# refresh-bio/KMC

Measured on NVIDIA H100. Metric: stage-2 k-mers/s (k=31), higher is better.
Workload: dtype u64

## Files before the change

kmc_b200/csrc/expand.cuh:

```cuda
#pragma once
#include "common.cuh"

#ifndef KMCB200_EXPAND_UNROLL
#define KMCB200_EXPAND_UNROLL 8
#endif

namespace kmcb {

constexpr int kExpandUnroll = KMCB200_EXPAND_UNROLL;

#ifndef KMCB200_EXPAND_IPT
#define KMCB200_EXPAND_IPT 8
#endif
template <int WORDS> struct ExpandCfg { static constexpr int kTile = WORDS == 1 ? 4096 : 2048, kThreads = WORDS == 1 ? 4096 / KMCB200_EXPAND_IPT : 256; };
constexpr int kExpandMinTile = 2048;

struct ExpandArgs {
	const uint8_t* bin;
	uint64_t size;
	const uint64_t* pack_start;
	uint32_t n_packs;
	uint32_t k;
	uint32_t min_rec_bytes;
	uint32_t tile;
	uint32_t both_strands;
	uint64_t n_rec;
	uint32_t* sk_off;
	uint32_t* sk_kpre;
	uint32_t* tile_first;
	uint32_t* pack_nsk;
	uint32_t* pack_nk;
	uint64_t* pack_kbase;
	uint32_t* pack_tbase;
	uint32_t* tile_pack;
	uint4* tile_desc;
	uint64_t tile_pack_cap;
	uint32_t* status;
	uint32_t* flags;
	void* recs;
	uint16_t* cells1;
	uint64_t* item_lo1;
	uint16_t* item_cnt1;
	uint32_t top_shift;
	uint32_t mode;
	uint32_t fshift, fprefix, fmask;
	uint64_t* hist12;
	unsigned long long* out_counter;
	const uint16_t* blk_of_prefix;
	const uint64_t* region_start;
	uint32_t n_blocks;
};
enum : uint32_t { kExpandAll = 0, kExpandCount12 = 1, kExpandFilter = 2, kExpandScatter = 3 };
constexpr uint32_t kExpandMaxBlocks = 512;
constexpr uint64_t kExpandUnknownRecs = ~0ull;

enum : uint32_t { kErrPackWalk = 1, kErrRecCount = 2 };
constexpr uint32_t kExpandAbortFlag = 2;

__device__ __forceinline__ uint64_t tile_first_base(uint64_t pack_start, uint32_t p, uint32_t tile) { return pack_start * 4 / tile + p; }

constexpr int kWalkSegBytes = 256;
constexpr int kWalkSegs = 256;
constexpr int kWalkChunk = kWalkSegBytes * kWalkSegs;
#ifndef KMCB200_WALK_SPEC
#define KMCB200_WALK_SPEC 1024
#endif
constexpr int kWalkSpec = KMCB200_WALK_SPEC;

__global__ void __launch_bounds__(kWalkSegs, 3) walk_packs_parallel_kernel(const ExpandArgs a, uint32_t* pack_done)
{
	extern __shared__ __align__(16) uint8_t wsm[];
	__shared__ uint32_t s_entry[kWalkSegs], s_exit[kWalkSegs], s_w[16];
	__shared__ uint32_t s_bad;
	const uint32_t p = blockIdx.x, tid = threadIdx.x, lane = tid & 31, warp = tid >> 5;
	const uint64_t pstart = a.pack_start[p];
	const uint32_t len = (uint32_t)min(a.pack_start[p + 1] - pstart, (uint64_t)kWalkChunk + 1);
	if (len > (uint32_t)kWalkChunk || len == 0) { if (tid == 0) pack_done[p] = len == 0 ? 1u : 0u; if (len == 0 && tid == 0) { a.pack_nsk[p] = 0; a.pack_nk[p] = 0; } return; }
	{
		const uintptr_t g0 = reinterpret_cast<uintptr_t>(a.bin + pstart);
		const uintptr_t g0a = g0 & ~(uintptr_t)15;
		const uint32_t shift = (uint32_t)(g0 - g0a);
		const uint32_t nvec = (len + shift + 15) >> 4;
		for (uint32_t v0 = tid; v0 < nvec; v0 += 8 * kWalkSegs) {
			uint4 r[8];
#pragma unroll
// ... 329 lines not shown
}

template <int WORDS>
__device__ __forceinline__ uint32_t rec_top_digit(const Rec<WORDS>& r, uint32_t shift)
{
	const uint32_t wi = shift >> 6, off = shift & 63u;
	uint64_t lo = r.w[0], hi = 0;
#pragma unroll
	for (int i = 1; i < WORDS; ++i) {
		if (wi == (uint32_t)i) lo = r.w[i];
		if (wi + 1 == (uint32_t)i) hi = r.w[i];
	}
	uint64_t v = lo >> off;
	if (WORDS > 1 && off) v |= hi << (64u - off);
	return (uint32_t)v & 0xFFu;
}

template <int WORDS>
__device__ __forceinline__ uint32_t msd_free_bits(const Rec<WORDS>& r, uint32_t shift, uint32_t mask)
{
	if (WORDS == 1) return (uint32_t)(r.w[0] >> shift) & mask;
	const uint32_t wi = shift >> 6, off = shift & 63u;
	uint64_t lo = r.w[0], hi = 0;
#pragma unroll
	for (int i = 1; i < WORDS; ++i) {
		if (wi == (uint32_t)i) lo = r.w[i];
		if (wi + 1 == (uint32_t)i) hi = r.w[i];
	}
	uint64_t v = lo >> off;
	if (off) v |= hi << (64u - off);
	return (uint32_t)v & mask;
}

template <int WORDS, uint32_t MODE = kExpandAll>
__global__ void __launch_bounds__(ExpandCfg<WORDS>::kThreads, WORDS <= 2 ? 2048 / ExpandCfg<WORDS>::kThreads : 6) expand_kernel(const ExpandArgs a)
{
	constexpr int kExpandTile = ExpandCfg<WORDS>::kTile, kExpandThreads = ExpandCfg<WORDS>::kThreads;
	constexpr int IPT = kExpandTile / kExpandThreads;
	constexpr int MAXSK = 1024, STAGE = 12288;
	constexpr int HW = kExpandTile / 32;
	__shared__ uint32_t hbits[HW];
	__shared__ uint32_t hpre[HW];
	__shared__ uint32_t s_bit[MAXSK];
	__shared__ __align__(16) uint8_t s_bytes[STAGE + 32];
	__shared__ uint32_t s_jmax;
	__shared__ unsigned long long s_fbase;
	__shared__ uint32_t warp_max[kExpandThreads / 32];
	__shared__ uint32_t htop[256];
	static_assert(HW <= 128 && HW % 32 == 0, "the head bitmap is scanned by one warp, HW / 32 words per lane");
	const uint32_t tid = threadIdx.x, lane = tid & 31, warp = tid >> 5;
	const uint32_t le_mask = 0xffffffffu >> (31u - lane);
	static_assert(kExpandThreads % 32 == 0, "output slot i * threads + tid belongs to lane tid % 32");
	if (tid < 256) htop[tid] = 0;
	const uint32_t total_tiles = a.status[1];
	Rec<WORDS>* __restrict__ out = reinterpret_cast<Rec<WORDS>*>(a.recs);

	for (uint32_t g = blockIdx.x; g < total_tiles; g += gridDim.x) {
		const uint4 da = __ldg(a.tile_desc + 2 * (size_t)g), db = __ldg(a.tile_desc + 2 * (size_t)g + 1);
		if (g + gridDim.x < total_tiles) asm volatile("prefetch.global.L2 [%0];" ::"l"(a.tile_desc + 2 * (size_t)(g + gridDim.x)));
		const uint64_t slot0 = da.x;
		const uint32_t nsk = da.y;
		const uint32_t j_lo = da.z;
		const uint32_t off_lo = da.w;
		const uint32_t tile_start = db.x & ~(uint32_t)(kExpandTile - 1);
		const uint32_t cnt = (db.x & (uint32_t)(kExpandTile - 1)) + 1u;
		const uint32_t* __restrict__ kpre = a.sk_kpre + slot0;
		const uint32_t* __restrict__ off = a.sk_off + slot0;
		const uintptr_t g0a = reinterpret_cast<uintptr_t>(a.bin + off_lo) & ~(uintptr_t)15;
		const uint32_t base_off = (uint32_t)(reinterpret_cast<uintptr_t>(a.bin + off_lo) - g0a);

		__syncthreads();
		if (tid < (uint32_t)HW) hbits[tid] = 0;
		if (tid == 0) s_jmax = j_lo;
		__syncthreads();
		{
			uint32_t jm = j_lo;
			for (uint32_t j = j_lo + tid; j < nsk; j += kExpandThreads) {
				const uint32_t kp = kpre[j];
				if (j > j_lo && kp >= tile_start + cnt) break;
				const uint32_t rel = j - j_lo;
				if (rel < (uint32_t)MAXSK) s_bit[rel] = 8u * (base_off + (off[j] - off_lo) + 1u) + 2u * tile_start - 2u * kp;
				if (j > j_lo) atomicOr(&hbits[(kp - tile_start) >> 5], 1u << ((kp - tile_start) & 31u));
				jm = j;
			}
			if (jm > j_lo) atomicMax(&s_jmax, jm);
		}
		__syncthreads();
		const uint32_t j_hi = s_jmax;
		const uint64_t b_hi = j_hi + 1 < nsk ? (uint64_t)off[j_hi + 1] : (uint64_t)db.y;
		const uint64_t span = reinterpret_cast<uintptr_t>(a.bin + b_hi) - g0a;
		const bool staged = (j_hi - j_lo) < (uint32_t)MAXSK && span + 16 <= (uint64_t)STAGE;
		if (staged)
			for (uint32_t v = tid; v * 16 < span + 8; v += kExpandThreads) {
				uint4 x = __ldg(reinterpret_cast<const uint4*>(g0a) + v);
				x.x = __byte_perm(x.x, 0, 0x0123); x.y = __byte_perm(x.y, 0, 0x0123); x.z = __byte_perm(x.z, 0, 0x0123); x.w = __byte_perm(x.w, 0, 0x0123);
				reinterpret_cast<uint4*>(s_bytes)[v] = x;
			}
		if (warp == 0) {
			constexpr int WPL = HW / 32;
			uint32_t c[WPL], tot = 0;
#pragma unroll
			for (int i = 0; i < WPL; ++i) { c[i] = __popc(hbits[lane * WPL + i]); tot += c[i]; }
			uint32_t inc = tot;
#pragma unroll
			for (int o = 1; o < 32; o <<= 1) {
				const uint32_t x = __shfl_up_sync(0xffffffffu, inc, o);
				if (lane >= (uint32_t)o) inc += x;
			}
			uint32_t ex = inc - tot;
#pragma unroll
			for (int i = 0; i < WPL; ++i) { hpre[lane * WPL + i] = ex; ex += c[i]; }
		}
		__syncthreads();

		const uint64_t obase = ((uint64_t)db.w << 32) | db.z;
		auto kmer_of = [&](uint32_t slot) -> Rec<WORDS> {
			const uint32_t rel = hpre[slot >> 5] + __popc(hbits[slot >> 5] & le_mask);
			if (staged) return extract_kmer_be32<WORDS>(reinterpret_cast<const uint32_t*>(s_bytes), s_bit[rel] + 2u * slot, a.k, a.both_strands != 0);
			const uint32_t j = j_lo + rel;
			const uint32_t s = tile_start + slot - kpre[j];
			return extract_kmer<WORDS>(a.bin + off[j] + 1, s, a.k, a.both_strands != 0,
				[](uintptr_t wa) { return __ldg(reinterpret_cast<const unsigned long long*>(wa)); });
		};
		if constexpr (MODE == kExpandAll) {
#pragma unroll kExpandUnroll
			for (int i = 0; i < IPT; ++i) {
				const uint32_t slot = i * kExpandThreads + tid;
				if (slot < cnt) {
					const Rec<WORDS> r = kmer_of(slot);
					out[obase + slot] = r;
					atomicAdd(&htop[rec_top_digit<WORDS>(r, a.top_shift)], 1u);
				}
			}
			__syncthreads();
			if (tid < 256) {
				a.cells1[(uint64_t)tid * total_tiles + g] = (uint16_t)htop[tid];
				htop[tid] = 0;
			}
			if (tid == 0) { a.item_lo1[g] = obase; a.item_cnt1[g] = (uint16_t)cnt; }
		} else if constexpr (MODE == kExpandCount12) {
			for (int i = 0; i < IPT; ++i) {
				const uint32_t slot = i * kExpandThreads + tid;
				if (slot < cnt) {
					const Rec<WORDS> r = kmer_of(slot);
					atomicAdd(reinterpret_cast<unsigned long long*>(a.hist12) + msd_free_bits<WORDS>(r, a.fshift, 0xFFFu), 1ull);
				}
			}
		} else if constexpr (MODE == kExpandScatter) {
			__shared__ uint32_t s_bcnt[kExpandMaxBlocks];
			__shared__ unsigned long long s_bbase[kExpandMaxBlocks];
			for (uint32_t b = tid; b < a.n_blocks; b += kExpandThreads) s_bcnt[b] = 0;
			__syncthreads();
			uint16_t blk[IPT], rnk[IPT];
#pragma unroll
			for (int i = 0; i < IPT; ++i) {
				const uint32_t slot = i * kExpandThreads + tid;
				if (slot < cnt) {
					const Rec<WORDS> r = kmer_of(slot);
					blk[i] = a.blk_of_prefix[msd_free_bits<WORDS>(r, a.fshift, 0xFFFu)];
					if (blk[i] != 0xFFFFu) rnk[i] = (uint16_t)atomicAdd(&s_bcnt[blk[i]], 1u);
				}
			}
			__syncthreads();
			for (uint32_t b = tid; b < a.n_blocks; b += kExpandThreads) {
				const uint32_t c = s_bcnt[b];
				if (c) s_bbase[b] = a.region_start[b] + atomicAdd(a.out_counter + b, (unsigned long long)c);
			}
			__syncthreads();
#pragma unroll
			for (int i = 0; i < IPT; ++i) {
				const uint32_t slot = i * kExpandThreads + tid;
				if (slot < cnt && blk[i] != 0xFFFFu) out[s_bbase[blk[i]] + rnk[i]] = kmer_of(slot);
// ... 25 lines not shown
```

kmc_b200/csrc/kmc_b200.cu:

```cuda
#include "../../include/kmc_b200.h"
#include "common.cuh"
#include "expand.cuh"
#include "expand_fused.cuh"
#include "radix_sort.cuh"
#include "count.cuh"
#include "msd_sort.cuh"
#include "leaf_warp.cuh"
#include "leaf_hash.cuh"
#include "leaf_hash_cta.cuh"
#include "leaf_hash_wide.cuh"
#include "split.cuh"
#include "fastx.cuh"
#include "small_k.cuh"

#include <cmath>
#include <cstddef>
#include <cstdarg>
#include <cstdio>
#include <cstdlib>
#include <cstring>
#include <string>
#include <vector>
#include <algorithm>
#include <list>
#include <thread>

using namespace kmcb;

namespace {

constexpr int kMaxPasses = 4 * 8;
constexpr int kHistRows = kMaxPasses + 1;
constexpr int kCounterSlots = kMaxPasses + 8;
constexpr uint32_t kEpochLimit = (1u << 22) - 2;
constexpr int kStageRing = 4;
constexpr size_t kMaxLeaves = 256 * 1024;
constexpr uint32_t kHeavyListCap = 2048;

thread_local std::string g_create_error;

enum { kHistNone = 0, kHistTiles = 1, kHistAligned = 2 };

struct ZeroBlock {
	uint64_t hist[kHistRows][256];
	uint32_t counters[kCounterSlots];
	uint32_t status[2];
	uint32_t msd_flags[4];
	uint32_t msd_n_items[2];
	uint32_t msd_counters[4];
	uint32_t pack_ticket[4];
	uint32_t heavy_count[2];
	uint32_t heavy_list[kHeavyListCap];
	uint32_t leaf_group_sum[kMaxLeaves / 1024];
};

static_assert(sizeof(ZeroBlock) % 4 == 0, "zeroed word by word");

struct Slot {
	cudaStream_t stream = nullptr;
	uint8_t* recs_a = nullptr; size_t recs_a_cap = 0;
	uint8_t* recs_b = nullptr; size_t recs_b_cap = 0;
	uint8_t* recs_x = nullptr; size_t recs_x_cap = 0;
	uint8_t* d_bin = nullptr; size_t bin_cap = 0;
	uint64_t* d_pack_start = nullptr; size_t packs_cap = 0;
	uint64_t* h_pack_start[kStageRing] = {}; cudaEvent_t ev_pack[kStageRing] = {}; int ring = 0;
	uint32_t* pack_nsk = nullptr; uint32_t* pack_nk = nullptr; uint32_t* pack_tbase = nullptr; uint64_t* pack_kbase = nullptr;
	uint32_t* pack_done = nullptr;
	uint32_t* sk_off = nullptr; size_t sk_off_cap = 0;
	uint32_t* sk_kpre = nullptr; size_t sk_kpre_cap = 0;
	uint32_t* tile_first = nullptr; size_t tile_first_cap = 0;
	uint32_t* tile_pack = nullptr; size_t tile_pack_cap = 0;
	uint4* tile_desc = nullptr; size_t tile_desc_cap = 0;
	ZeroBlock* zero = nullptr;
	uint64_t* desc = nullptr; size_t desc_cap = 0;
	uint64_t* msd_seg1 = nullptr;
	uint64_t* msd_start2 = nullptr;
	uint64_t* msd_start3 = nullptr;
	uint32_t* msd_item_base1 = nullptr;
	uint32_t* msd_item_base2 = nullptr;
	uint32_t* msd_item_seg2 = nullptr; size_t msd_item_seg2_cap = 0;
	uint64_t* msd_item_lo1 = nullptr; size_t msd_item_lo1_cap = 0;
	uint16_t* msd_item_cnt1 = nullptr; size_t msd_item_cnt1_cap = 0;
	uint16_t* msd_cells = nullptr; size_t msd_cells_cap = 0;
	uint32_t* msd_cell_scan = nullptr; size_t msd_cell_scan_cap = 0;
	uint32_t* msd_block_sums = nullptr; size_t msd_block_sums_cap = 0;
	uint8_t* leaf_tmp = nullptr; size_t leaf_tmp_cap = 0;
	uint32_t* leaf_emit = nullptr; uint64_t* leaf_off = nullptr;
	const char* pass_names[kMaxPasses + 8] = {};
	uint32_t last_n_packs = 1;
	uint64_t* cdesc = nullptr; size_t cdesc_cap = 0;
	uint64_t* pdesc = nullptr; size_t pdesc_cap = 0;
	int hist_mode = 0;
	uint8_t* d_out = nullptr; size_t out_cap = 0;
	uint64_t* d_lut = nullptr;
	uint64_t* d_result = nullptr; uint64_t* h_result = nullptr; uint64_t* h_result_dev = nullptr;
	cudaEvent_t ev_begin = nullptr, ev_expand = nullptr, ev_sort = nullptr, ev_count = nullptr, ev_result = nullptr;
	cudaEvent_t ev_h2d = nullptr, ev_done = nullptr, ev_walk = nullptr;
	cudaEvent_t ev_pass[kMaxPasses + 8] = {};
	int n_passes_run = 0;
	bool ran_expand = false, ran_sort = false, ran_count = false;
	uint64_t* d_hist12 = nullptr; unsigned long long* d_out_counter = nullptr; size_t out_counter_cap = 0;
	uint16_t* d_blk_of_prefix = nullptr; uint64_t* d_region_start = nullptr; size_t region_cap = 0; bool last_scatter = false;
	uint64_t* tot_lut = nullptr; uint64_t* tot_res = nullptr; uint32_t last_blocks = 0;
	bool scan_lut = false; uint64_t scan_base = 0;
	uint8_t* d_extras = nullptr; size_t extras_cap = 0; uint64_t* d_pack_rec = nullptr; size_t pack_rec_cap = 0;
	uint64_t* h_pack_rec = nullptr; size_t h_pack_rec_cap = 0; bool have_extras = false;
	bool sync_done = false; uint64_t sync_out_bytes = 0; uint64_t sync_stats[4] = {};
	bool busy = false;
	uint8_t* host_out = nullptr; uint64_t host_out_cap = 0; uint64_t* host_lut = nullptr; uint64_t pending_n_rec = 0;
};

}

struct kmcb200_ctx {
	kmcb200_params prm{};
	int words = 1;
	uint32_t key_bytes = 0, suffix_bytes = 0, counter_bytes = 0;
	uint64_t lut_entries = 0;
	int sm_count = 0;
	int occ_radix = 1, occ_expand = 1, occ_msd_part = 1, occ_msd_part_wide = 1, occ_msd_local = 1;
	uint32_t force_b2 = 0;
	bool use_msd = true;
	bool use_fused = false;
	bool scatter_blocks = true;
	uint64_t key_block_records = 1ull << 28;
	bool overlap_walk = true;
	bool use_leaf = true;
	int occ_leaf = 1;
	int occ_leaf_hash = 1;
	bool leaf_hash_wide = true;
	bool leaf_hash = true;
	int leaf_cta = 2;
	int leaf_cta_warps = 4, leaf_cta_slot_bits = 12;
	int occ_leaf_cta = 1;
	uint32_t leaf_max_b2 = 8;
	uint32_t leaf_target = 1024;
	uint32_t leaf_fill_pct = 62;
	uint32_t leaf_ratio0_q8 = 90;
	uint64_t max_block_records = 1ull << 28;
	uint64_t max_chunk_bytes = 1ull << 30;
	uint32_t leaf_round_pct = 100;
	int leaf_slot_bits = 10;
	uint32_t epoch = 1;
	uint64_t launches = 0;
	cudaStream_t compute = nullptr;
	std::vector<Slot> slots;
	std::string err;
};

namespace {

int fail(kmcb200_ctx* c, int code, const char* fmt, ...)
{
// ... 53 lines not shown
	size_t n = std::max<size_t>(need_elems + need_elems / 8, 1024);
	if (p) CU(cudaFree(p));
	p = nullptr; cap = 0;
	CU(cudaMalloc(reinterpret_cast<void**>(&p), n * sizeof(T) + 256));
	if (zero) { CU(cudaMemset(p, 0, n * sizeof(T) + 256)); CU(cudaDeviceSynchronize()); }
	cap = n;
	return 0;
}

int next_epoch(kmcb200_ctx* ctx, uint32_t* out, uint32_t count = 1)
{
	if (ctx->epoch + count >= kEpochLimit) {
		CU(cudaDeviceSynchronize());
		for (auto& s : ctx->slots) {
			if (s.desc) CU(cudaMemset(s.desc, 0, s.desc_cap * sizeof(uint64_t)));
			if (s.cdesc) CU(cudaMemset(s.cdesc, 0, s.cdesc_cap * sizeof(uint64_t)));
			if (s.pdesc) CU(cudaMemset(s.pdesc, 0, s.pdesc_cap * sizeof(uint64_t)));
		}
		CU(cudaDeviceSynchronize());
		ctx->epoch = 1;
	}
	*out = ctx->epoch;
	ctx->epoch += count;
	return 0;
}

template <int WORDS>
int setup_kernels(kmcb200_ctx* ctx)
{
	CU(cudaFuncSetAttribute(radix_pass_kernel<WORDS>, cudaFuncAttributeMaxDynamicSharedMemorySize, SortSmem<WORDS>::kBytes));
	CU(cudaFuncSetAttribute(lsd_sort_kernel<WORDS>, cudaFuncAttributeMaxDynamicSharedMemorySize, SortSmem<WORDS>::kBytes));
	CU(cudaOccupancyMaxActiveBlocksPerMultiprocessor(&ctx->occ_radix, lsd_sort_kernel<WORDS>, SortCfg<WORDS>::kThreads, SortSmem<WORDS>::kBytes));
	CU(cudaOccupancyMaxActiveBlocksPerMultiprocessor(&ctx->occ_expand, expand_kernel<WORDS>, ExpandCfg<WORDS>::kThreads, 0));
	CU(cudaFuncSetAttribute(expand_fused_kernel<WORDS>, cudaFuncAttributeMaxDynamicSharedMemorySize, FxSmem<WORDS>::kBytes));
	const size_t cs = count_smem_bytes<WORDS>(ctx->suffix_bytes + ctx->counter_bytes);
	CU(cudaFuncSetAttribute(count_emit_kernel<WORDS>, cudaFuncAttributeMaxDynamicSharedMemorySize, (int)cs));
	CU(cudaFuncSetAttribute(msd_partition_kernel<WORDS>, cudaFuncAttributeMaxDynamicSharedMemorySize, MsdSmem<WORDS>::kBytes));
	CU(cudaOccupancyMaxActiveBlocksPerMultiprocessor(&ctx->occ_msd_part, msd_partition_kernel<WORDS>, MsdCfg<WORDS>::kThreads + 32, MsdSmem<WORDS>::kBytes));
	CU(cudaFuncSetAttribute(msd_partition_kernel<WORDS, 1024>, cudaFuncAttributeMaxDynamicSharedMemorySize, MsdSmem<WORDS, 1024>::kBytes));
	CU(cudaOccupancyMaxActiveBlocksPerMultiprocessor(&ctx->occ_msd_part_wide, msd_partition_kernel<WORDS, 1024>, MsdCfg<WORDS>::kThreads + 32, MsdSmem<WORDS, 1024>::kBytes));
	if (ctx->occ_msd_part_wide < 1) ctx->occ_msd_part_wide = 1;
	const int local_smem = msd_local_cap<WORDS>() * 8 * WORDS + (MsdLocalCfg<WORDS>::kThreads / 32) * 1024;
	CU(cudaFuncSetAttribute(msd_local_sort_kernel<WORDS>, cudaFuncAttributeMaxDynamicSharedMemorySize, local_smem));
	CU(cudaOccupancyMaxActiveBlocksPerMultiprocessor(&ctx->occ_msd_local, msd_local_sort_kernel<WORDS>, MsdLocalCfg<WORDS>::kThreads, local_smem));
	if (ctx->occ_radix < 1) ctx->occ_radix = 1;
	if (ctx->occ_expand < 1) ctx->occ_expand = 1;
	if (ctx->occ_msd_part < 1) ctx->occ_msd_part = 1;
	if (ctx->occ_msd_local < 1) ctx->occ_msd_local = 1;
	return 0;
}

template <int WORDS>
int launch_expand(kmcb200_ctx* ctx, const ExpandArgs& a, cudaStream_t st)
{
	const uint64_t n_bound = a.n_rec == kExpandUnknownRecs ? a.size * 4 : a.n_rec;
	const uint32_t max_tiles = (uint32_t)(n_bound / ExpandCfg<WORDS>::kTile) + a.n_packs + 1;
	const uint32_t grid = std::min<uint32_t>(max_tiles, (uint32_t)(ctx->sm_count * ctx->occ_expand));
	switch (a.mode) {
	case kExpandAll: expand_kernel<WORDS, kExpandAll><<<grid, ExpandCfg<WORDS>::kThreads, 0, st>>>(a); break;
	case kExpandCount12: expand_kernel<WORDS, kExpandCount12><<<grid, ExpandCfg<WORDS>::kThreads, 0, st>>>(a); break;
	case kExpandScatter: expand_kernel<WORDS, kExpandScatter><<<grid, ExpandCfg<WORDS>::kThreads, 0, st>>>(a); break;
	default: expand_kernel<WORDS, kExpandFilter><<<grid, ExpandCfg<WORDS>::kThreads, 0, st>>>(a); break;
	}
	ctx->launches++;
	CU(cudaGetLastError());
	return 0;
}

__global__ void msd_setup_kernel(uint64_t* seg1, uint32_t* item_base1, uint32_t* n_items1, uint64_t n, uint32_t tile)
{
	seg1[0] = 0; seg1[1] = n;
	const uint32_t nt = (uint32_t)((n + tile - 1) / tile);
	item_base1[0] = 0; item_base1[1] = nt;
	*n_items1 = nt;
}

template <int WORDS>
uint32_t choose_b2(const kmcb200_ctx* ctx, uint64_t n, bool counted_leaves)
{
	auto bits_for = [&](uint64_t target) { uint32_t lg = 0; while ((1ull << lg) < (n + target - 1) / target) ++lg; return lg > 8 ? lg - 8 : 0u; };
	uint32_t b2;
	if (counted_leaves) {
		b2 = std::min(bits_for(1024), 10u);
		if (WORDS == 1 && b2 > 8 && !ctx->leaf_hash) b2 = std::max(8u, std::min(bits_for(2048), 10u));
		if (WORDS == 1 && b2 > 8 && ctx->leaf_hash) b2 = std::max(8u, std::min(bits_for(ctx->leaf_target), ctx->leaf_max_b2));
		if (ctx->force_b2) b2 = ctx->force_b2;
	} else
		b2 = std::min(bits_for(std::max<uint64_t>(msd_local_cap<WORDS>() / 5, 64)), 8u);
	return b2;
}
template <int WORDS> uint32_t choose_nd2(const kmcb200_ctx* ctx, uint64_t n, bool counted_leaves) { return 1u << choose_b2<WORDS>(ctx, n, counted_leaves); }

// ... 21 lines not shown
	cell_reduce_kernel<<<nb, 256, 0, st>>>(s.msd_cells, n_items, nd, s.msd_block_sums, flags);
	cell_scan_sums_kernel<<<1, 1024, 0, st>>>(s.msd_block_sums, n_items, nd, flags);
	cell_scan_kernel<<<nb, 256, 0, st>>>(s.msd_cells, n_items, nd, s.msd_block_sums, s.msd_cell_scan, flags);
	ctx->launches += 3;
	CU(cudaGetLastError());
	return 0;
}

template <int WORDS>
int launch_lsd_sort(kmcb200_ctx* ctx, Slot& s, void* in, void* out, uint64_t n, uint32_t key_bytes, const uint32_t* run_flag, uint32_t run_need,
	uint64_t* reset_lut, uint64_t* reset_result, cudaStream_t st)
{
	constexpr int TILE = SortSmem<WORDS>::kTile;
	LsdSortArgs a{};
	a.a = in; a.b = out; a.n = n; a.n_tiles = (uint32_t)((n + TILE - 1) / TILE); a.key_bytes = key_bytes;
	a.hist = &s.zero->hist[0][0]; a.desc = s.desc; a.tile_counters = s.zero->counters;
	if (int rc = next_epoch(ctx, &a.epoch0, key_bytes)) return rc;
	a.run_flag = run_flag; a.run_need = run_need;
	a.reset_lut = reset_lut; a.reset_lut_entries = ctx->lut_entries; a.reset_result = reset_result;
	const uint32_t grid = std::max(1u, std::min<uint32_t>(a.n_tiles, (uint32_t)(ctx->sm_count * ctx->occ_radix)));
	void* params[] = {&a};
	CU(cudaLaunchCooperativeKernel(reinterpret_cast<const void*>(lsd_sort_kernel<WORDS>), dim3(grid), dim3(SortCfg<WORDS>::kThreads), params, SortSmem<WORDS>::kBytes, st));
	ctx->launches++;
	return 0;
}

struct LeafPlan {
	bool active = false;
	const void* recs = nullptr;
	const uint64_t* start = nullptr;
	uint32_t n_leaves = 0, low_bits = 0;
};

template <int WORDS>
int launch_sort(kmcb200_ctx* ctx, Slot& s, void* a, void* b, uint64_t n, uint32_t key_bytes, uint32_t key_bits, int hist_mode, uint32_t n_packs, cudaStream_t st, bool* result_in_b, LeafPlan* plan = nullptr)
{
	constexpr int TILE = SortSmem<WORDS>::kTile;
	constexpr int MTILE = msd_tile<WORDS>();
	const uint64_t n_tiles64 = (n + TILE - 1) / TILE;
	if (n_tiles64 > 0x7fffffffull || n >= (1ull << 32)) return fail(ctx, KMCB200_ERR_INVALID, "bin too large: %llu records", (unsigned long long)n);
	const uint32_t n_tiles = (uint32_t)n_tiles64;
	const bool msd = ctx->use_msd && key_bits >= 24 && n >= (1u << 16);
	const uint32_t top_shift = key_bits - 8;
	if (int rc = ensure(ctx, s.desc, s.desc_cap, (size_t)n_tiles * 256, true)) return rc;
	if (msd) if (int rc = ensure_msd<WORDS>(ctx, s, n, n_packs, choose_nd2<WORDS>(ctx, n, plan != nullptr))) return rc;

	const bool hist_ready = hist_mode == kHistTiles;
	if (hist_mode == kHistNone) if (int rc = zero_async(ctx, s.zero, sizeof(ZeroBlock), st)) return rc;
	int iv = 0;
	CU(cudaEventRecord(s.ev_pass[0], st));
	void* lsd_in = a; void* lsd_out = b;
	const uint32_t* lsd_flag = nullptr;
	if (msd) {
		const uint32_t b2 = choose_b2<WORDS>(ctx, n, plan != nullptr);
		const uint32_t nd2 = 1u << b2;
		const uint32_t cap = plan ? (WORDS == 1 ? kLwMaxHeavyLeaf : kLwMaxLeaf) : (uint32_t)msd_local_cap<WORDS>();
		const bool final_in_b = (key_bytes % 2) == 0;
		void* fin = final_in_b ? b : a;
		uint32_t* flags = s.zero->msd_flags;
		const uint32_t* never = &flags[1];
		const size_t max_items1 = hist_ready ? msd_max_items1(n, n_packs) : (size_t)(n / MTILE) + 2;
		const size_t max_items2 = (size_t)(n / MTILE) + 260;
		const uint32_t pgrid1 = (uint32_t)std::min<size_t>(max_items1, (size_t)ctx->sm_count * ctx->occ_msd_part);
		const uint32_t pgrid2 = (uint32_t)std::min<size_t>(max_items2, (size_t)ctx->sm_count * (nd2 > 256 ? ctx->occ_msd_part_wide : ctx->occ_msd_part));
		const int local_smem = msd_local_cap<WORDS>() * 8 * WORDS + (MsdLocalCfg<WORDS>::kThreads / 32) * 1024;

		MsdItems items1{};
		if (hist_ready) {
			items1.item_lo = s.msd_item_lo1; items1.item_cnt = s.msd_item_cnt1; items1.n_items = &s.zero->status[1];
		} else if (hist_mode == kHistAligned) {
			items1.seg_start = s.msd_seg1; items1.item_base = s.msd_item_base1; items1.item_seg = s.msd_item_seg2; items1.n_items = s.msd_item_base1 + 1;
		} else {
			msd_setup_kernel<<<1, 1, 0, st>>>(s.msd_seg1, s.msd_item_base1, &s.zero->msd_n_items[0], n, MTILE);
			items1.seg_start = s.msd_seg1; items1.item_base = s.msd_item_base1; items1.item_seg = s.msd_item_seg2 ;
			items1.n_items = &s.zero->msd_n_items[0];
			if (int rc = zero_async(ctx, s.msd_item_seg2, max_items1 * sizeof(uint32_t), st)) return rc;
			MsdCountArgs c1{a, items1, top_shift, 256, s.msd_cells, never};
			msd_count_kernel<WORDS><<<(uint32_t)std::min<size_t>(max_items1, (size_t)ctx->sm_count * 4), 512, 0, st>>>(c1);
			ctx->launches += 2;
		}
		if (int rc = launch_cell_scan(ctx, s, items1.n_items, 256, max_items1, never, st)) return rc;
		s.pass_names[iv] = "msd_scan_L1"; CU(cudaEventRecord(s.ev_pass[++iv], st));
		MsdBoundsArgs b1{};
		b1.cell_scan = s.msd_cell_scan; b1.items = items1; b1.S = 1; b1.nd = 256; b1.n = n; b1.start = s.msd_start2;
		b1.cap = b2 == 0 ? cap : 0; b1.flags = flags;
		b1.tile = b2 > 0 ? MTILE : 0; b1.item_base = s.msd_item_base2; b1.item_seg = s.msd_item_seg2; b1.n_items = &s.zero->msd_n_items[1];
		MsdPartArgs p1{};
		p1.in = a; p1.out = b; p1.items = items1; p1.cell_scan = s.msd_cell_scan; p1.shift = top_shift; p1.nd = 256;
		p1.flags = never;
		msd_partition_kernel<WORDS><<<pgrid1, MsdCfg<WORDS>::kThreads + 32, MsdSmem<WORDS>::kBytes, st>>>(p1);
		s.pass_names[iv] = "msd_partition_L1"; CU(cudaEventRecord(s.ev_pass[++iv], st));
		msd_bounds_kernel<<<1, 1024, 0, st>>>(b1);
		ctx->launches += 2;
		if (b2 > 0) {
			MsdItems items2{};
			items2.seg_start = s.msd_start2; items2.item_base = s.msd_item_base2; items2.item_seg = s.msd_item_seg2; items2.n_items = &s.zero->msd_n_items[1];
			MsdCountArgs c2{b, items2, top_shift - b2, nd2, s.msd_cells, flags};
			if (nd2 > 512) msd_count_kernel<WORDS, 1024><<<(uint32_t)std::min<size_t>(max_items2, (size_t)ctx->sm_count * 4), 512, 0, st>>>(c2);
			else if (nd2 > 256) msd_count_kernel<WORDS, 512><<<(uint32_t)std::min<size_t>(max_items2, (size_t)ctx->sm_count * 4), 512, 0, st>>>(c2);
			else msd_count_kernel<WORDS><<<(uint32_t)std::min<size_t>(max_items2, (size_t)ctx->sm_count * 4), 512, 0, st>>>(c2);
			ctx->launches++;
			if (int rc = launch_cell_scan(ctx, s, items2.n_items, nd2, max_items2, flags, st)) return rc;
			MsdBoundsArgs bb{};
			bb.cell_scan = s.msd_cell_scan; bb.items = items2; bb.S = 256; bb.nd = nd2; bb.n = n; bb.start = s.msd_start3; bb.cap = cap; bb.flags = flags; bb.tile = 0;
			msd_bounds_flat_kernel<<<(256 * nd2 + 256) / 256 + 1, 256, 0, st>>>(bb);
			ctx->launches++;
			s.pass_names[iv] = "msd_count_L2"; CU(cudaEventRecord(s.ev_pass[++iv], st));
			MsdPartArgs p2{};
			p2.in = b; p2.out = a; p2.items = items2; p2.cell_scan = s.msd_cell_scan; p2.shift = top_shift - b2; p2.nd = nd2;
			p2.flags = flags;
			if (nd2 > 256) msd_partition_kernel<WORDS, 1024><<<pgrid2, MsdCfg<WORDS>::kThreads + 32, MsdSmem<WORDS, 1024>::kBytes, st>>>(p2);
			else msd_partition_kernel<WORDS><<<pgrid2, MsdCfg<WORDS>::kThreads + 32, MsdSmem<WORDS>::kBytes, st>>>(p2);
			ctx->launches++;
			s.pass_names[iv] = "msd_partition_L2"; CU(cudaEventRecord(s.ev_pass[++iv], st));
		}
		if (plan) {
			plan->active = true;
			plan->recs = b2 > 0 ? a : b; plan->start = b2 > 0 ? s.msd_start3 : s.msd_start2; plan->n_leaves = 256 * nd2; plan->low_bits = top_shift - b2;
		} else {
			MsdLocalArgs lo{};
			lo.in = b2 > 0 ? a : b; lo.out = fin; lo.start = b2 > 0 ? s.msd_start3 : s.msd_start2; lo.n_buckets = 256 * nd2;
			lo.low_bits = top_shift - b2; lo.bucket_counter = &s.zero->msd_counters[2]; lo.flags = flags;
			const uint32_t lgrid = (uint32_t)std::min<size_t>(lo.n_buckets, (size_t)ctx->sm_count * ctx->occ_msd_local);
			msd_local_sort_kernel<WORDS><<<lgrid, MsdLocalCfg<WORDS>::kThreads, local_smem, st>>>(lo);
			ctx->launches++;
			s.pass_names[iv] = "msd_local_sort"; CU(cudaEventRecord(s.ev_pass[++iv], st));
// ... 115 lines not shown
	if (fused) {
		st = st_expand;
		const uint32_t nd2 = DISPATCH_WORDS(ctx, choose_nd2, ctx, n_rec, ctx->use_leaf);
		if (int rc = DISPATCH_WORDS(ctx, ensure_msd, ctx, s, n_rec, np, nd2)) return rc;
		if (int rc = ensure(ctx, s.pdesc, s.pdesc_cap, (size_t)np + 1, true)) return rc;
		const uint32_t mtile = ctx->words == 1 ? (uint32_t)msd_tile<1>() : (uint32_t)msd_tile<2>();
		static_assert(msd_tile<2>() == msd_tile<3>() && msd_tile<2>() == msd_tile<4>(), "one tile size for all wide records");
		const uint32_t n_tiles = (uint32_t)((n_rec + mtile - 1) / mtile);
		uint32_t tile_shift = 0;
		while ((1u << tile_shift) < mtile) ++tile_shift;
		InitExtra x;
		x.cells = reinterpret_cast<uint32_t*>(s.msd_cells); x.cell_words = ((size_t)256 * n_tiles + 1) / 2;
		x.item_seg = s.msd_item_seg2; x.item_seg_words = (size_t)n_tiles + 2;
		x.seg1 = s.msd_seg1; x.item_base1 = s.msd_item_base1; x.n = n_rec; x.n_tiles = n_tiles;
		bin_init_kernel<<<296, 256, 0, st>>>(reinterpret_cast<uint32_t*>(s.zero), (uint32_t)(sizeof(ZeroBlock) / 4), reinterpret_cast<uint32_t*>(zero_lut),
			(size_t)ctx->lut_entries * 2, reinterpret_cast<uint32_t*>(zero_result), x);
		FusedArgs f{};
		f.bin = d_bin; f.size = size; f.pack_start = s.d_pack_start; f.n_packs = np; f.k = k; f.both_strands = ctx->prm.both_strands; f.n_rec = n_rec;
		f.recs = d_recs; f.cells1 = reinterpret_cast<uint32_t*>(s.msd_cells); f.n_tiles = n_tiles; f.tile_shift = tile_shift;
		f.top_shift = std::max(2u * k, 8u) - 8u;
		f.desc = s.pdesc; f.ticket = &s.zero->pack_ticket[0]; f.status = s.zero->status; f.flags = s.zero->msd_flags;
		if (int rc = next_epoch(ctx, &f.epoch)) return rc;
		switch (ctx->words) {
		case 1: expand_fused_kernel<1><<<np, kFxThreads, FxSmem<1>::kBytes, st>>>(f); break;
		case 2: expand_fused_kernel<2><<<np, kFxThreads, FxSmem<2>::kBytes, st>>>(f); break;
		case 3: expand_fused_kernel<3><<<np, kFxThreads, FxSmem<3>::kBytes, st>>>(f); break;
		default: expand_fused_kernel<4><<<np, kFxThreads, FxSmem<4>::kBytes, st>>>(f); break;
		}
		ctx->launches += 2;
		CU(cudaGetLastError());
		s.hist_mode = kHistAligned;
		return 0;
	}
	s.hist_mode = em.mode == kExpandAll ? kHistTiles : kHistNone;

	if (int rc = ensure(ctx, s.sk_off, s.sk_off_cap, size / min_rec + 2)) return rc;
	if (int rc = ensure(ctx, s.sk_kpre, s.sk_kpre_cap, size / min_rec + 2)) return rc;
	if (int rc = ensure(ctx, s.tile_first, s.tile_first_cap, size * 4 / kExpandMinTile + np + 2)) return rc;
	const uint64_t n_bound = n_rec == kExpandUnknownRecs ? size * 4 : n_rec;
	if (int rc = ensure(ctx, s.tile_pack, s.tile_pack_cap, n_bound / kExpandMinTile + np + 2)) return rc;
	if (int rc = ensure(ctx, s.tile_desc, s.tile_desc_cap, 2 * (n_bound / kExpandMinTile + np + 2))) return rc;

	ExpandArgs a;
	a.bin = d_bin; a.size = size; a.pack_start = s.d_pack_start; a.n_packs = np; a.k = k; a.min_rec_bytes = min_rec;
	a.both_strands = ctx->prm.both_strands; a.n_rec = n_rec;
	a.tile = ctx->words == 1 ? ExpandCfg<1>::kTile : ExpandCfg<2>::kTile;
	a.sk_off = s.sk_off; a.sk_kpre = s.sk_kpre; a.tile_first = s.tile_first; a.pack_nsk = s.pack_nsk; a.pack_nk = s.pack_nk;
	a.pack_kbase = s.pack_kbase; a.pack_tbase = s.pack_tbase; a.tile_pack = s.tile_pack; a.tile_pack_cap = n_bound / kExpandMinTile + np + 2;
	a.tile_desc = s.tile_desc;
	a.status = s.zero->status; a.flags = s.zero->msd_flags;
	a.recs = d_recs;
	a.mode = em.mode; a.fshift = em.fshift; a.fprefix = em.fprefix; a.fmask = em.fmask; a.hist12 = em.hist12; a.out_counter = em.out_counter;
	a.blk_of_prefix = em.blk_of_prefix; a.region_start = em.region_start; a.n_blocks = em.n_blocks;
	if (em.mode == kExpandAll) {
		if (int rc = DISPATCH_WORDS(ctx, ensure_msd, ctx, s, n_rec, np, DISPATCH_WORDS(ctx, choose_nd2, ctx, n_rec, ctx->use_leaf))) return rc;
		a.cells1 = s.msd_cells; a.item_lo1 = s.msd_item_lo1; a.item_cnt1 = s.msd_item_cnt1;
	} else { a.cells1 = nullptr; a.item_lo1 = nullptr; a.item_cnt1 = nullptr; }
	a.top_shift = std::max(2u * k, 8u) - 8u;

	bin_init_kernel<<<64, 256, 0, st>>>(reinterpret_cast<uint32_t*>(s.zero), (uint32_t)(sizeof(ZeroBlock) / 4), reinterpret_cast<uint32_t*>(zero_lut),
		(size_t)ctx->lut_entries * 2, reinterpret_cast<uint32_t*>(zero_result), InitExtra());
	if (s.have_extras && em.mode == kExpandAll) {
		index_from_extras_kernel<<<np, 1024, 0, st>>>(a, s.d_extras, s.d_pack_rec);
		ctx->launches += 2;
		big_pack = false;
	} else {
		walk_packs_parallel_kernel<<<np, kWalkSegs, kWalkChunk + 32, st>>>(a, s.pack_done);
		ctx->launches += 2;
	}
	if (big_pack) {
		walk_packs_kernel<<<(np + kWalkWarpsPerBlock - 1) / kWalkWarpsPerBlock, 32 * kWalkWarpsPerBlock, 0, st>>>(a, s.pack_done);
		ctx->launches++;
	}
	scan_packs_kernel<<<1, 1024, 0, st>>>(a);
	tile_desc_kernel<<<(uint32_t)((a.tile_pack_cap + 255) / 256), 256, 0, st>>>(a);
	ctx->launches += 2;
	CU(cudaGetLastError());
	if (st_expand != st) {
		CU(cudaEventRecord(s.ev_walk, st));
		CU(cudaStreamWaitEvent(st_expand, s.ev_walk, 0));
	}
	return DISPATCH_WORDS(ctx, launch_expand, ctx, a, st_expand);
}

int stage_count(kmcb200_ctx* ctx, Slot& s, const void* sorted, uint64_t n, uint8_t* d_out, uint64_t out_capacity,
	uint64_t* d_lut, uint64_t* d_result, cudaStream_t st, bool outputs_zeroed = false, bool guarded = false, const uint64_t* out_base = nullptr)
{
	if (!outputs_zeroed) {
		bin_init_kernel<<<64, 256, 0, st>>>(&s.zero->counters[kMaxPasses], 1u, reinterpret_cast<uint32_t*>(d_lut), (size_t)ctx->lut_entries * 2, reinterpret_cast<uint32_t*>(d_result), InitExtra());
		ctx->launches++;
		CU(cudaGetLastError());
	}
	if (n == 0) return 0;
	return DISPATCH_WORDS(ctx, launch_count, ctx, s, sorted, n, d_out, out_capacity, d_lut, d_result, guarded ? &s.zero->msd_flags[1] : nullptr, 0u, st, out_base);
}
// ... 156 lines not shown
		if (int rc = DISPATCH_SLOTS(ctx, launch_heavy_leaves, WORDS, ctx, la, st)) return rc;
	}
	leaf_scan_kernel<<<(plan.n_leaves + 1023) / 1024, 1024, 0, st>>>(s.leaf_emit, s.zero->leaf_group_sum, plan.n_leaves, s.leaf_off, d_result, out_capacity, ob, flags, out_base);
	leaf_gather_kernel<<<(plan.n_leaves + 7) / 8, 256, 0, st>>>(s.leaf_tmp, plan.start, s.leaf_emit, s.leaf_off, plan.n_leaves, ob, d_out, d_result, flags, out_base);
	ctx->launches += 2;
	int iv = s.n_passes_run;
	s.pass_names[iv] = "leaf_count"; CU(cudaEventRecord(s.ev_pass[++iv], st));
	if (int rc = launch_lsd_sort<WORDS>(ctx, s, rb, ra, n_rec, ctx->key_bytes, flags, kMsdFlagFallback, d_lut, d_result, st)) return rc;
	s.pass_names[iv] = "lsd_fallback(all passes)"; CU(cudaEventRecord(s.ev_pass[++iv], st));
	s.n_passes_run = iv;
	CU(cudaEventRecord(s.ev_sort, st));
	s.ran_sort = true;
	const void* sorted = (ctx->key_bytes % 2 == 0) ? rb : ra;
	return launch_count<WORDS>(ctx, s, sorted, n_rec, d_out, out_capacity, d_lut, d_result, flags, kMsdFlagFallback, st, out_base);
}

int run_bin(kmcb200_ctx* ctx, Slot& s, const uint8_t* d_bin, uint64_t size, uint64_t n_rec, const uint64_t* pack_bytes, uint32_t n_packs,
	uint8_t* d_out, uint64_t out_capacity, uint64_t* d_lut, uint64_t* d_result, cudaStream_t st, bool packs_uploaded = false, uint64_t* host_result = nullptr,
	cudaStream_t st_walk = nullptr)
{
	const size_t rec_bytes = (size_t)ctx->words * 8;
	s.ran_expand = s.ran_sort = s.ran_count = false;
	CU(cudaEventRecord(s.ev_begin, st));
	if (n_rec == 0 || size == 0) {
		if (n_rec != 0 || size != 0) return fail(ctx, KMCB200_ERR_BIN_FORMAT, "bin with size=%llu but n_rec=%llu", (unsigned long long)size, (unsigned long long)n_rec);
		if (int rc = stage_count(ctx, s, nullptr, 0, d_out, out_capacity, d_lut, d_result, st)) return rc;
		if (host_result) { finish_result_kernel<<<1, 32, 0, st>>>(d_result, 0, nullptr, nullptr, host_result); ctx->launches++; }
		CU(cudaEventRecord(s.ev_expand, st)); CU(cudaEventRecord(s.ev_sort, st)); CU(cudaEventRecord(s.ev_count, st));
		s.n_passes_run = 0;
		return 0;
	}
	if (int rc = ensure(ctx, s.recs_a, s.recs_a_cap, n_rec * rec_bytes)) return rc;
	if (int rc = ensure(ctx, s.recs_b, s.recs_b_cap, n_rec * rec_bytes)) return rc;
	if (int rc = stage_expand(ctx, s, d_bin, size, n_rec, pack_bytes, n_packs, s.recs_a, st, ExpandMode(), packs_uploaded, d_lut, d_result, st_walk)) return rc;
	CU(cudaEventRecord(s.ev_expand, st));
	s.ran_expand = true;
	bool in_b = false;
	const uint32_t np_eff = (n_packs && pack_bytes) ? n_packs : 1u;
	if (ctx->use_leaf) {
		if (int rc = DISPATCH_WORDS(ctx, run_sort_count_leaves, ctx, s, n_rec, np_eff, d_out, out_capacity, d_lut, d_result, st, false, 0u, 0u, true)) return rc;
	} else {
		if (int rc = DISPATCH_WORDS(ctx, launch_sort, ctx, s, s.recs_a, s.recs_b, n_rec, ctx->key_bytes, 2u * ctx->prm.kmer_len, s.hist_mode, np_eff, st, &in_b)) return rc;
		CU(cudaEventRecord(s.ev_sort, st));
		s.ran_sort = true;
		const void* sorted = in_b ? s.recs_b : s.recs_a;
		if (int rc = stage_count(ctx, s, sorted, n_rec, d_out, out_capacity, d_lut, d_result, st, true, true)) return rc;
	}
	finish_result_kernel<<<1, 32, 0, st>>>(d_result, n_rec, s.zero->status, s.zero->msd_flags, host_result);
	ctx->launches++;
	CU(cudaEventRecord(s.ev_count, st));
	s.ran_count = true;
	return 0;
}

struct BinChunk { uint32_t pack0, npacks; uint64_t byte0, bytes, dev_off; };
struct KeyBlock { uint32_t prefix, bits; uint64_t n; };

__global__ void accumulate_block_kernel(uint64_t* tot_lut, const uint64_t* blk_lut, uint64_t lut_entries, uint64_t* tot_res, const uint64_t* blk_res,
	const unsigned long long* appended, uint64_t expected)
{
	for (uint64_t i = (uint64_t)blockIdx.x * blockDim.x + threadIdx.x; i < lut_entries; i += (uint64_t)gridDim.x * blockDim.x) tot_lut[i] += blk_lut[i];
	if (blockIdx.x == 0 && threadIdx.x == 0) {
		tot_res[0] += blk_res[0]; tot_res[1] += blk_res[1]; tot_res[2] += blk_res[2];
		tot_res[5] |= blk_res[5]; tot_res[7] |= blk_res[7];
		if (appended && *appended != expected) tot_res[6] |= kErrRecCount;
		tot_res[4] += blk_res[4];
	}
// ... 823 lines not shown
```

Baseline: 24.17 billion.

## Fuse level-1 MSD partition into a second k-mer expansion pass

For one-word records on the MSD path, the first expansion pass now only builds the per-tile top-digit histogram and writes no records. The level-1 MSD partition kernel is replaced by a second expansion pass that re-extracts k-mers, sorts them locally by top digit in shared memory, and scatters them straight to their partitioned positions. This removes one full write and read of the record array, in exchange for decoding the k-mers twice and using more shared memory at lower occupancy in the partition kernel. The cell-counting pass also gets a shortcut that reads only the top byte from the staged bits.

```diff
diff --git a/kmc_b200/csrc/expand.cuh b/kmc_b200/csrc/expand.cuh
--- a/kmc_b200/csrc/expand.cuh
+++ b/kmc_b200/csrc/expand.cuh
@@ -42,6 +42,7 @@
 	uint64_t* item_lo1;
 	uint16_t* item_cnt1;
 	uint32_t top_shift;
+	const uint32_t* cell_scan;
 	uint32_t mode;
 	uint32_t fshift, fprefix, fmask;
 	uint64_t* hist12;
@@ -50,7 +51,8 @@
 	const uint64_t* region_start;
 	uint32_t n_blocks;
 };
-enum : uint32_t { kExpandAll = 0, kExpandCount12 = 1, kExpandFilter = 2, kExpandScatter = 3 };
+enum : uint32_t { kExpandAll = 0, kExpandCount12 = 1, kExpandFilter = 2, kExpandScatter = 3, kExpandCells = 4, kExpandPartition = 5 };
+template <int WORDS> __host__ __device__ constexpr bool expand_partition_supported() { return WORDS == 1; }
 constexpr uint32_t kExpandMaxBlocks = 512;
 constexpr uint64_t kExpandUnknownRecs = ~0ull;
 
@@ -446,17 +448,22 @@
 	return (uint32_t)v & mask;
 }
 
+template <int WORDS, uint32_t MODE>
+__host__ __device__ constexpr int expand_min_blocks() { return MODE == kExpandPartition ? 3 : WORDS <= 2 ? 2048 / ExpandCfg<WORDS>::kThreads : 6; }
+
 template <int WORDS, uint32_t MODE = kExpandAll>
-__global__ void __launch_bounds__(ExpandCfg<WORDS>::kThreads, WORDS <= 2 ? 2048 / ExpandCfg<WORDS>::kThreads : 6) expand_kernel(const ExpandArgs a)
+__global__ void __launch_bounds__(ExpandCfg<WORDS>::kThreads, expand_min_blocks<WORDS, MODE>()) expand_kernel(const ExpandArgs a)
 {
 	constexpr int kExpandTile = ExpandCfg<WORDS>::kTile, kExpandThreads = ExpandCfg<WORDS>::kThreads;
 	constexpr int IPT = kExpandTile / kExpandThreads;
 	constexpr int MAXSK = 1024, STAGE = 12288;
 	constexpr int HW = kExpandTile / 32;
+	constexpr int SBYTES = MODE == kExpandPartition && kExpandTile * 8 * WORDS > STAGE + 32 ? kExpandTile * 8 * WORDS : STAGE + 32;
+	static_assert(MODE != kExpandPartition || expand_partition_supported<WORDS>(), "kExpandPartition: one-word records only");
 	__shared__ uint32_t hbits[HW];
 	__shared__ uint32_t hpre[HW];
 	__shared__ uint32_t s_bit[MAXSK];
-	__shared__ __align__(16) uint8_t s_bytes[STAGE + 32];
+	__shared__ __align__(16) uint8_t s_bytes[SBYTES];
 	__shared__ uint32_t s_jmax;
 	__shared__ unsigned long long s_fbase;
 	__shared__ uint32_t warp_max[kExpandThreads / 32];
@@ -465,11 +472,16 @@
 	const uint32_t tid = threadIdx.x, lane = tid & 31, warp = tid >> 5;
 	const uint32_t le_mask = 0xffffffffu >> (31u - lane);
 	static_assert(kExpandThreads % 32 == 0, "output slot i * threads + tid belongs to lane tid % 32");
+	if constexpr (MODE == kExpandPartition)
+		if (a.flags[1] & kExpandAbortFlag) return;
 	if (tid < 256) htop[tid] = 0;
 	const uint32_t total_tiles = a.status[1];
 	Rec<WORDS>* __restrict__ out = reinterpret_cast<Rec<WORDS>*>(a.recs);
 
 	for (uint32_t g = blockIdx.x; g < total_tiles; g += gridDim.x) {
+		uint32_t digit_base = 0;
+		if constexpr (MODE == kExpandPartition)
+			if (tid < 256) digit_base = __ldg(a.cell_scan + g + (size_t)tid * total_tiles);
 		const uint4 da = __ldg(a.tile_desc + 2 * (size_t)g), db = __ldg(a.tile_desc + 2 * (size_t)g + 1);
 		if (g + gridDim.x < total_tiles) asm volatile("prefetch.global.L2 [%0];" ::"l"(a.tile_desc + 2 * (size_t)(g + gridDim.x)));
 		const uint64_t slot0 = da.x;
@@ -536,14 +548,28 @@
 			return extract_kmer<WORDS>(a.bin + off[j] + 1, s, a.k, a.both_strands != 0,
 				[](uintptr_t wa) { return __ldg(reinterpret_cast<const unsigned long long*>(wa)); });
 		};
-		if constexpr (MODE == kExpandAll) {
+		auto top_digit_of = [&](uint32_t slot) -> uint32_t {
+			if (WORDS > 1 || !staged || a.top_shift + 8u != 2u * a.k) return rec_top_digit<WORDS>(kmer_of(slot), a.top_shift);
+			const uint32_t rel = hpre[slot >> 5] + __popc(hbits[slot >> 5] & le_mask);
+			const uint32_t B = s_bit[rel] + 2u * slot;
+			const uint32_t* sw = reinterpret_cast<const uint32_t*>(s_bytes);
+			auto byte_at = [&](uint32_t b) { const uint32_t wi = b >> 5; return __funnelshift_l(sw[wi + 1], sw[wi], b & 31u) >> 24; };
+			const uint32_t f = byte_at(B);
+			if (!a.both_strands) return f;
+			uint32_t r = ~byte_at(B + 2u * a.k - 8u) & 0xFFu;
+			r = ((r & 0x03u) << 6) | ((r & 0x0Cu) << 2) | ((r & 0x30u) >> 2) | ((r & 0xC0u) >> 6);
+			return min(f, r);
+		};
+		if constexpr (MODE == kExpandAll || MODE == kExpandCells) {
 #pragma unroll kExpandUnroll
 			for (int i = 0; i < IPT; ++i) {
 				const uint32_t slot = i * kExpandThreads + tid;
 				if (slot < cnt) {
-					const Rec<WORDS> r = kmer_of(slot);
-					out[obase + slot] = r;
-					atomicAdd(&htop[rec_top_digit<WORDS>(r, a.top_shift)], 1u);
+					if constexpr (MODE == kExpandAll) {
+						const Rec<WORDS> r = kmer_of(slot);
+						out[obase + slot] = r;
+						atomicAdd(&htop[rec_top_digit<WORDS>(r, a.top_shift)], 1u);
+					} else atomicAdd(&htop[top_digit_of(slot)], 1u);
 				}
 			}
 			__syncthreads();
@@ -552,6 +578,55 @@
 				htop[tid] = 0;
 			}
 			if (tid == 0) { a.item_lo1[g] = obase; a.item_cnt1[g] = (uint16_t)cnt; }
+		} else if constexpr (MODE == kExpandPartition) {
+			__shared__ uint32_t s_excl[256], s_goff[256];
+			Rec<WORDS> key[IPT];
+			uint32_t rank[IPT / 2] = {};
+#pragma unroll
+			for (int i = 0; i < IPT; ++i) {
+				const uint32_t slot = i * kExpandThreads + tid;
+				if (slot < cnt) {
+					key[i] = kmer_of(slot);
+					rank[i / 2] |= atomicAdd(&htop[rec_top_digit<WORDS>(key[i], a.top_shift)], 1u) << (16 * (i & 1));
+				}
+			}
+			__syncthreads();
+			uint32_t c = 0, inc = 0;
+			if (tid < 256) {
+				c = htop[tid];
+				htop[tid] = 0;
+				inc = c;
+#pragma unroll
+				for (int o = 1; o < 32; o <<= 1) {
+					const uint32_t x = __shfl_up_sync(0xffffffffu, inc, o);
+					if (lane >= (uint32_t)o) inc += x;
+				}
+				if (lane == 31) warp_max[warp] = inc;
+			}
+			__syncthreads();
+			if (tid < 256) {
+				uint32_t ex = inc - c;
+#pragma unroll
+				for (int w = 0; w < 8; ++w) if ((uint32_t)w < warp) ex += warp_max[w];
+				s_excl[tid] = ex;
+				s_goff[tid] = digit_base - ex;
+			}
+			__syncthreads();
+			Rec<WORDS>* buf = reinterpret_cast<Rec<WORDS>*>(s_bytes);
+#pragma unroll
+			for (int i = 0; i < IPT; ++i) {
+				const uint32_t slot = i * kExpandThreads + tid;
+				if (slot < cnt) buf[s_excl[rec_top_digit<WORDS>(key[i], a.top_shift)] + ((rank[i / 2] >> (16 * (i & 1))) & 0xFFFFu)] = key[i];
+			}
+			__syncthreads();
+#pragma unroll
+			for (int i = 0; i < IPT; ++i) {
+				const uint32_t q = i * kExpandThreads + tid;
+				if (q < cnt) {
+					const Rec<WORDS> r = buf[q];
+					out[s_goff[rec_top_digit<WORDS>(r, a.top_shift)] + q] = r;
+				}
+			}
 		} else if constexpr (MODE == kExpandCount12) {
 			for (int i = 0; i < IPT; ++i) {
 				const uint32_t slot = i * kExpandThreads + tid;
diff --git a/kmc_b200/csrc/kmc_b200.cu b/kmc_b200/csrc/kmc_b200.cu
--- a/kmc_b200/csrc/kmc_b200.cu
+++ b/kmc_b200/csrc/kmc_b200.cu
@@ -39,7 +39,7 @@
 
 thread_local std::string g_create_error;
 
-enum { kHistNone = 0, kHistTiles = 1, kHistAligned = 2 };
+enum { kHistNone = 0, kHistTiles = 1, kHistAligned = 2, kHistCells = 3 };
 
 struct ZeroBlock {
 	uint64_t hist[kHistRows][256];
@@ -91,6 +91,7 @@
 	uint64_t* cdesc = nullptr; size_t cdesc_cap = 0;
 	uint64_t* pdesc = nullptr; size_t pdesc_cap = 0;
 	int hist_mode = 0;
+	ExpandArgs expand_args{};
 	uint8_t* d_out = nullptr; size_t out_cap = 0;
 	uint64_t* d_lut = nullptr;
 	uint64_t* d_result = nullptr; uint64_t* h_result = nullptr; uint64_t* h_result_dev = nullptr;
@@ -118,7 +119,7 @@
 	uint32_t key_bytes = 0, suffix_bytes = 0, counter_bytes = 0;
 	uint64_t lut_entries = 0;
 	int sm_count = 0;
-	int occ_radix = 1, occ_expand = 1, occ_msd_part = 1, occ_msd_part_wide = 1, occ_msd_local = 1;
+	int occ_radix = 1, occ_expand = 1, occ_expand_part = 1, occ_msd_part = 1, occ_msd_part_wide = 1, occ_msd_local = 1;
 	uint32_t force_b2 = 0;
 	bool use_msd = true;
 	bool use_fused = false;
@@ -238,6 +239,8 @@
 	CU(cudaFuncSetAttribute(lsd_sort_kernel<WORDS>, cudaFuncAttributeMaxDynamicSharedMemorySize, SortSmem<WORDS>::kBytes));
 	CU(cudaOccupancyMaxActiveBlocksPerMultiprocessor(&ctx->occ_radix, lsd_sort_kernel<WORDS>, SortCfg<WORDS>::kThreads, SortSmem<WORDS>::kBytes));
 	CU(cudaOccupancyMaxActiveBlocksPerMultiprocessor(&ctx->occ_expand, expand_kernel<WORDS>, ExpandCfg<WORDS>::kThreads, 0));
+	if constexpr (expand_partition_supported<WORDS>())
+		CU((cudaOccupancyMaxActiveBlocksPerMultiprocessor(&ctx->occ_expand_part, expand_kernel<WORDS, kExpandPartition>, ExpandCfg<WORDS>::kThreads, 0)));
 	CU(cudaFuncSetAttribute(expand_fused_kernel<WORDS>, cudaFuncAttributeMaxDynamicSharedMemorySize, FxSmem<WORDS>::kBytes));
 	const size_t cs = count_smem_bytes<WORDS>(ctx->suffix_bytes + ctx->counter_bytes);
 	CU(cudaFuncSetAttribute(count_emit_kernel<WORDS>, cudaFuncAttributeMaxDynamicSharedMemorySize, (int)cs));
@@ -261,9 +264,16 @@
 {
 	const uint64_t n_bound = a.n_rec == kExpandUnknownRecs ? a.size * 4 : a.n_rec;
 	const uint32_t max_tiles = (uint32_t)(n_bound / ExpandCfg<WORDS>::kTile) + a.n_packs + 1;
-	const uint32_t grid = std::min<uint32_t>(max_tiles, (uint32_t)(ctx->sm_count * ctx->occ_expand));
+	const uint32_t grid = std::min<uint32_t>(max_tiles, (uint32_t)(ctx->sm_count * (a.mode == kExpandPartition ? std::max(ctx->occ_expand_part, 1) : ctx->occ_expand)));
 	switch (a.mode) {
 	case kExpandAll: expand_kernel<WORDS, kExpandAll><<<grid, ExpandCfg<WORDS>::kThreads, 0, st>>>(a); break;
+	case kExpandCells:
+	case kExpandPartition:
+		if constexpr (expand_partition_supported<WORDS>()) {
+			if (a.mode == kExpandCells) expand_kernel<WORDS, kExpandCells><<<grid, ExpandCfg<WORDS>::kThreads, 0, st>>>(a);
+			else expand_kernel<WORDS, kExpandPartition><<<grid, ExpandCfg<WORDS>::kThreads, 0, st>>>(a);
+			break;
+		} else return fail(ctx, KMCB200_ERR_INVALID, "no level-1 partition expansion for %d-word records", WORDS);
 	case kExpandCount12: expand_kernel<WORDS, kExpandCount12><<<grid, ExpandCfg<WORDS>::kThreads, 0, st>>>(a); break;
 	case kExpandScatter: expand_kernel<WORDS, kExpandScatter><<<grid, ExpandCfg<WORDS>::kThreads, 0, st>>>(a); break;
 	default: expand_kernel<WORDS, kExpandFilter><<<grid, ExpandCfg<WORDS>::kThreads, 0, st>>>(a); break;
@@ -351,6 +361,8 @@
 	uint32_t n_leaves = 0, low_bits = 0;
 };
 
+bool msd_path(const kmcb200_ctx* ctx, uint64_t n, uint32_t key_bits) { return ctx->use_msd && key_bits >= 24 && n >= (1u << 16); }
+
 template <int WORDS>
 int launch_sort(kmcb200_ctx* ctx, Slot& s, void* a, void* b, uint64_t n, uint32_t key_bytes, uint32_t key_bits, int hist_mode, uint32_t n_packs, cudaStream_t st, bool* result_in_b, LeafPlan* plan = nullptr)
 {
@@ -359,12 +371,13 @@
 	const uint64_t n_tiles64 = (n + TILE - 1) / TILE;
 	if (n_tiles64 > 0x7fffffffull || n >= (1ull << 32)) return fail(ctx, KMCB200_ERR_INVALID, "bin too large: %llu records", (unsigned long long)n);
 	const uint32_t n_tiles = (uint32_t)n_tiles64;
-	const bool msd = ctx->use_msd && key_bits >= 24 && n >= (1u << 16);
+	const bool msd = msd_path(ctx, n, key_bits);
+	if (hist_mode == kHistCells && !msd) return fail(ctx, KMCB200_ERR_INVALID, "the records of this bin were not expanded");
 	const uint32_t top_shift = key_bits - 8;
 	if (int rc = ensure(ctx, s.desc, s.desc_cap, (size_t)n_tiles * 256, true)) return rc;
 	if (msd) if (int rc = ensure_msd<WORDS>(ctx, s, n, n_packs, choose_nd2<WORDS>(ctx, n, plan != nullptr))) return rc;
 
-	const bool hist_ready = hist_mode == kHistTiles;
+	const bool hist_ready = hist_mode == kHistTiles || hist_mode == kHistCells;
 	if (hist_mode == kHistNone) if (int rc = zero_async(ctx, s.zero, sizeof(ZeroBlock), st)) return rc;
 	int iv = 0;
 	CU(cudaEventRecord(s.ev_pass[0], st));
@@ -407,10 +420,19 @@
 		MsdPartArgs p1{};
 		p1.in = a; p1.out = b; p1.items = items1; p1.cell_scan = s.msd_cell_scan; p1.shift = top_shift; p1.nd = 256;
 		p1.flags = never;
-		msd_partition_kernel<WORDS><<<pgrid1, MsdCfg<WORDS>::kThreads + 32, MsdSmem<WORDS>::kBytes, st>>>(p1);
-		s.pass_names[iv] = "msd_partition_L1"; CU(cudaEventRecord(s.ev_pass[++iv], st));
+		if (hist_mode == kHistCells) {
+			ExpandArgs ea = s.expand_args;
+			ea.mode = kExpandPartition; ea.recs = b; ea.cell_scan = s.msd_cell_scan;
+			if (int rc = launch_expand<WORDS>(ctx, ea, st)) return rc;
+			s.pass_names[iv] = "expand_scatter_L1";
+		} else {
+			msd_partition_kernel<WORDS><<<pgrid1, MsdCfg<WORDS>::kThreads + 32, MsdSmem<WORDS>::kBytes, st>>>(p1);
+			ctx->launches++;
+			s.pass_names[iv] = "msd_partition_L1";
+		}
+		CU(cudaEventRecord(s.ev_pass[++iv], st));
 		msd_bounds_kernel<<<1, 1024, 0, st>>>(b1);
-		ctx->launches += 2;
+		ctx->launches++;
 		if (b2 > 0) {
 			MsdItems items2{};
 			items2.seg_start = s.msd_start2; items2.item_base = s.msd_item_base2; items2.item_seg = s.msd_item_seg2; items2.n_items = &s.zero->msd_n_items[1];
@@ -592,7 +614,8 @@
 		s.hist_mode = kHistAligned;
 		return 0;
 	}
-	s.hist_mode = em.mode == kExpandAll ? kHistTiles : kHistNone;
+	const bool cells = em.mode == kExpandAll || em.mode == kExpandCells;
+	s.hist_mode = em.mode == kExpandAll ? kHistTiles : em.mode == kExpandCells ? kHistCells : kHistNone;
 
 	if (int rc = ensure(ctx, s.sk_off, s.sk_off_cap, size / min_rec + 2)) return rc;
 	if (int rc = ensure(ctx, s.sk_kpre, s.sk_kpre_cap, size / min_rec + 2)) return rc;
@@ -612,15 +635,17 @@
 	a.recs = d_recs;
 	a.mode = em.mode; a.fshift = em.fshift; a.fprefix = em.fprefix; a.fmask = em.fmask; a.hist12 = em.hist12; a.out_counter = em.out_counter;
 	a.blk_of_prefix = em.blk_of_prefix; a.region_start = em.region_start; a.n_blocks = em.n_blocks;
-	if (em.mode == kExpandAll) {
+	if (cells) {
 		if (int rc = DISPATCH_WORDS(ctx, ensure_msd, ctx, s, n_rec, np, DISPATCH_WORDS(ctx, choose_nd2, ctx, n_rec, ctx->use_leaf))) return rc;
 		a.cells1 = s.msd_cells; a.item_lo1 = s.msd_item_lo1; a.item_cnt1 = s.msd_item_cnt1;
 	} else { a.cells1 = nullptr; a.item_lo1 = nullptr; a.item_cnt1 = nullptr; }
 	a.top_shift = std::max(2u * k, 8u) - 8u;
+	a.cell_scan = nullptr;
+	if (em.mode == kExpandCells) s.expand_args = a;
 
 	bin_init_kernel<<<64, 256, 0, st>>>(reinterpret_cast<uint32_t*>(s.zero), (uint32_t)(sizeof(ZeroBlock) / 4), reinterpret_cast<uint32_t*>(zero_lut),
 		(size_t)ctx->lut_entries * 2, reinterpret_cast<uint32_t*>(zero_result), InitExtra());
-	if (s.have_extras && em.mode == kExpandAll) {
+	if (s.have_extras && cells) {
 		index_from_extras_kernel<<<np, 1024, 0, st>>>(a, s.d_extras, s.d_pack_rec);
 		ctx->launches += 2;
 		big_pack = false;
@@ -843,7 +868,9 @@
 	}
 	if (int rc = ensure(ctx, s.recs_a, s.recs_a_cap, n_rec * rec_bytes)) return rc;
 	if (int rc = ensure(ctx, s.recs_b, s.recs_b_cap, n_rec * rec_bytes)) return rc;
-	if (int rc = stage_expand(ctx, s, d_bin, size, n_rec, pack_bytes, n_packs, s.recs_a, st, ExpandMode(), packs_uploaded, d_lut, d_result, st_walk)) return rc;
+	ExpandMode em;
+	if (expand_partition_supported<1>() && ctx->words == 1 && !ctx->use_fused && n_rec < (1ull << 32) && msd_path(ctx, n_rec, 2u * ctx->prm.kmer_len)) em.mode = kExpandCells;
+	if (int rc = stage_expand(ctx, s, d_bin, size, n_rec, pack_bytes, n_packs, s.recs_a, st, em, packs_uploaded, d_lut, d_result, st_walk)) return rc;
 	CU(cudaEventRecord(s.ev_expand, st));
 	s.ran_expand = true;
 	bool in_b = false;
```

Result: faster. 25.13 billion, median of 6 (+4.0%).
